# ska-telescope/ska-sdp-screen-fitting

Hardware: AMD Instinct MI355X
Metric: screen-slots/sec (ant×time×freq) + FITS-cube wall-clock, KL 256² screen (higher is better)
Workload: dtype f64

## Files before the change

### include/screenfit.h

```cpp
#ifndef SCREENFIT_H
#define SCREENFIT_H

#include <stddef.h>
#include <stdint.h>

#ifdef __cplusplus
extern "C" {
#endif

#define SF_OK 0
#define SF_EINVAL (-22)
#define SF_ENOMEM (-12)
#define SF_EIO (-5)
#define SF_ENODEV (-19)

#define SF_MAX_DIR 60
#define SF_MAX_FIT_DIR 128
#define SF_MAX_EVAL_DIR 128

#define SF_SCREEN_PHASE 0
#define SF_SCREEN_TEC 1
#define SF_SCREEN_AMPLITUDE 2

#define SF_EVAL_NAN_SCRUB 1u
// ... 32 lines not shown
#define SF_OPT_EVAL_XCD_MAP 7
#define SF_OPT_EVAL_GROUPS 8
#define SF_OPT_EVAL_BANDS 9
#define SF_OPT_FIT_LEAN 10
#define SF_OPT_TESS_SLOTS 11
#define SF_OPT_TESS_WAVES 12
#define SF_OPT_TESS_TILE 13
#define SF_OPT_TESS_BOX 14
#define SF_OPT_EVAL_INT 15
#define SF_OPT_EVAL_WG_WAVES 16
#define SF_OPT_FIT_EIG_WAVES 17
#define SF_OPT_FIT_SUBSET_DELETION 18
#define SF_OPT_FIT_WIDE_CACHE 19
#define SF_OPT_FIT_WIDE_POOL_MB 20
#define SF_OPT_FIT_WIDE_POOL_MAX 21
#define SF_EVAL_KERNEL_AUTO 0
#define SF_EVAL_KERNEL_TILE 1
#define SF_EVAL_KERNEL_LDS4 2
#define SF_EVAL_KERNEL_LDS8 3
#define SF_EVAL_KERNEL_LDS16 4
#define SF_EVAL_KERNEL_LDS8H 5
#define SF_EVAL_KERNEL_LDS16H 6
#define SF_EVAL_KERNEL_TILE3 7
#define SF_EVAL_KERNEL_SHB 8
#define SF_EVAL_KERNEL_WIDE 9
int sf_get_eval_kernel(sf_ctx* ctx, int gain, unsigned flags, int* kernel);
#define SF_EVAL_CONTRACTION_F64 0
#define SF_EVAL_CONTRACTION_I8_DIGITS 1
int sf_get_eval_contraction(sf_ctx* ctx, int gain, unsigned flags, int* contraction);
int sf_set_option(sf_ctx* ctx, int option, int value);
// ... 6 lines not shown
                 double beta);
int sf_set_basis_wide(sf_ctx* ctx, const double* pp_host, int D, double r0,
                      double beta);
int sf_get_basis(sf_ctx* ctx, double* c_host, double* pinv_c_host,
                 double* u_host, double* eig_host);

int sf_set_piercepoints(sf_ctx* ctx, const double* pp_host, int D, double r0,
                        double beta);

int sf_kl_fit(sf_ctx* ctx, const double* phase, const float* weight, int T,
              int F, int A, const int* station_order_host,
              const sf_fit_params* params, double* coef, double* resid,
              float* w_out, int32_t* order_out);

int sf_get_fit_stats(sf_ctx* ctx, int* n_masks, int* n_general);

int sf_get_fit_pool(sf_ctx* ctx, uint64_t* masks_host, double* entries_host,
                    int max_masks, int* n_masks);
int sf_get_fit_pool_wide(sf_ctx* ctx, uint64_t* masks_host, double* entries_host,
                         int max_masks, int* n_masks);

int sf_set_grid(sf_ctx* ctx, const double* x_host, int nx,
                const double* y_host, int ny);

int sf_kl_eval(sf_ctx* ctx, const double* coef, int64_t S, float* out,
               int64_t ring_slots, unsigned flags);

int sf_kl_eval_gain(sf_ctx* ctx, const double* coef_phase,
                    const double* coef_xx, const double* coef_yy, int64_t S,
                    float* out, int64_t ring_slots, unsigned flags);
// ... 33 lines not shown
```

### ska-sdp-screen-fitting_amd/csrc/capi.hip

```cpp
#include <hip/hip_runtime.h>

#include <algorithm>
#include <cmath>
#include <cstring>
#include <string>
#include <vector>

#include "sf_internal.h"

namespace sf {
static thread_local std::string g_last_error;
void set_error(const std::string& msg) { g_last_error = msg; }
}

using sf::set_error;

namespace {

int check_device(int device) {
  int n = 0;
  hipError_t e = hipGetDeviceCount(&n);
  if (e != hipSuccess || n == 0) {
    set_error("no HIP device available");
    return SF_ENODEV;
// ... 103 lines not shown
  hipFree(ctx->d_cfrag);
  hipFree(ctx->d_pxy);
  hipFree(ctx->d_pfrag);
  hipFree(ctx->d_cdig);
  hipFree(ctx->d_kdig);
  hipFree(ctx->d_kflag);
  if (ctx->kdig_read) (void)hipEventDestroy(ctx->kdig_read);
  hipFree(ctx->d_skip);
  hipFree(ctx->d_st_order);
  hipFree(ctx->d_keys);
  hipFree(ctx->d_ids);
  hipFree(ctx->d_pool_mask);
  hipFree(ctx->d_pool);
  hipFree(ctx->d_pool_status);
  hipFree(ctx->d_pos);
  hipFree(ctx->d_sigma);
  hipFree(ctx->d_class);
  hipFree(ctx->d_counters);
  hipFree(ctx->d_scratch);
  hipFree(ctx->d_wscratch);
  hipFree(ctx->d_oscratch);
  hipFree(ctx->d_gw);
  hipFree(ctx->d_smooth);
  hipFree(ctx->d_tess_tab);
  hipFree(ctx->d_tec_ch);
  hipFree(ctx->d_trash);
  delete ctx;
  return SF_OK;
}

// ... 46 lines not shown
  SF_REQUIRE(ctx, SF_EINVAL, "sf_set_option: NULL context");
  switch (option) {
    case SF_OPT_FIT_GENERAL:
      ctx->force_general = value != 0;
      return SF_OK;
    case SF_OPT_EVAL_KERNEL:
      SF_REQUIRE(value >= SF_EVAL_KERNEL_AUTO && value <= SF_EVAL_KERNEL_WIDE,
                 SF_EINVAL, "sf_set_option: unknown evaluation kernel");
      ctx->eval_kernel = value;
      return SF_OK;
    case SF_OPT_FIT_PACK:
      ctx->fit_pack = value != 0;
      return SF_OK;
    case SF_OPT_FIT_LEAN:
      ctx->fit_lean = value != 0;
      return SF_OK;
    case SF_OPT_EVAL_KS_PAD:
      SF_REQUIRE(value >= 0 && value <= 3, SF_EINVAL,
                 "sf_set_option: k-step padding must be 0..3");
      ctx->eval_ks_pad = value;
      return SF_OK;
    case SF_OPT_EVAL_SLEEP:
      SF_REQUIRE(value >= 0 && value <= 1000, SF_EINVAL,
                 "sf_set_option: eval sleep must be 0..1000");
      ctx->eval_sleep = value;
      return SF_OK;
    case SF_OPT_EVAL_XCD_MAP:
      SF_REQUIRE(value >= -1 && value <= 1, SF_EINVAL,
                 "sf_set_option: XCD map must be -1, 0 or 1");
      ctx->eval_xcd_map = value;
// ... 273 lines not shown
}

int sf_get_fit_stats(sf_ctx* ctx, int* n_masks, int* n_general) {
  SF_REQUIRE(ctx, SF_EINVAL, "sf_get_fit_stats: NULL context");
  int c[sf::kFitCounters] = {};
  SF_HIP(hipSetDevice(ctx->device));
  SF_HIP(hipStreamSynchronize(ctx->stream));
  if (ctx->d_counters)
    SF_HIP(hipMemcpy(c, ctx->d_counters, sizeof(c), hipMemcpyDeviceToHost));
  static_assert(sf::kCntIds == sf::kCntWideDecomp, "n_masks reads one slot");
  if (n_masks) *n_masks = c[sf::kCntIds];
  if (n_general) *n_general = c[sf::kCntSlow];
  return SF_OK;
}

int sf_get_fit_pool(sf_ctx* ctx, uint64_t* masks_host, double* entries_host,
                    int max_masks, int* n_masks) {
  SF_REQUIRE(ctx && n_masks && max_masks >= 0, SF_EINVAL, "sf_get_fit_pool: bad argument");
  SF_REQUIRE(max_masks == 0 || (masks_host && entries_host), SF_EINVAL,
             "sf_get_fit_pool: NULL output");
  SF_REQUIRE(!ctx->wide, SF_EINVAL,
             "sf_get_fit_pool: 64-bit mask keys; above SF_MAX_DIR directions "
             "(sf_set_basis_wide) call sf_get_fit_pool_wide");
  SF_HIP(hipSetDevice(ctx->device));
  SF_HIP(hipStreamSynchronize(ctx->stream));
  int c0 = 0;
  if (ctx->d_counters)
    SF_HIP(hipMemcpy(&c0, ctx->d_counters + sf::kCntIds, sizeof(int),
                     hipMemcpyDeviceToHost));
  const int n = ctx->pool_D == ctx->D && (size_t)c0 <= ctx->pool_cap ? c0 : 0;
// ... 392 lines not shown
```

### ska-sdp-screen-fitting_amd/csrc/kl_fit_fast.hip

```cpp
#include <hip/hip_runtime.h>

#include <cmath>
#include <cstdlib>

#include "kl_fit_pool.h"
#include "kl_fit_steps.h"
#include "sf_internal.h"

namespace sf {

constexpr size_t kLdsBytes = 160 * 1024;
constexpr double kTinyW = kPinvAtol * 1.001;

template <int GW>
__global__ __launch_bounds__(256) void kl_classify_kernel(
    const float* __restrict__ weight, int64_t S, int F, int A, int D,
    const int* __restrict__ st_order, const uint8_t* __restrict__ skip,
    int ref_skip, unsigned long long* __restrict__ keys, int cap,
    int* __restrict__ pos, uint8_t* __restrict__ cls,
    int* __restrict__ counters,
    double* __restrict__ coef, double* __restrict__ resid,
    float* __restrict__ w_out, int32_t* __restrict__ order_out) {
  constexpr int kPerWave = 64 / GW;
  const int l = lane();
// ... 227 lines not shown

#ifndef SF_FIT_MINW
#define SF_FIT_MINW 4
#endif
template <bool SLOW, int SPW, bool LEAN>
__global__ __launch_bounds__(256, SLOW ? 1 : SF_FIT_MINW) void kl_fit_pass_kernel(
    int it, int niter, int64_t S, int F, int A, int D,
    const double* __restrict__ phase, const double* __restrict__ refph,
    int ref_sub, const double* __restrict__ g_u, const double* __restrict__ g_c,
    const double* __restrict__ g_eig, const int* __restrict__ st_order,
    const uint8_t* __restrict__ cls, int* __restrict__ pos,
    const int* __restrict__ ids, unsigned long long* __restrict__ keys, int cap,
    const double* __restrict__ pool, int pool_cap, int* __restrict__ counters,
    int screen_type, double nsigma, int adjust_order, double* __restrict__ coef,
    double* __restrict__ resid, float* __restrict__ w_out,
    int32_t* __restrict__ order_out) {
#pragma clang fp contract(off)
  extern __shared__ double smem[];
  const int ld = odd_ld(D);
  using G = Group<SPW>;
  using M = FitMath<!SLOW>;
  const G tm;
  constexpr bool CG = SPW == 1;
  const int nwaves = blockDim.x / 64;
  const int nslots = nwaves * SPW;
  const int wv = (threadIdx.x / 64) * SPW + G::index();
  const int d = G::lane();
  double* sU = smem;
  double* sC = CG ? nullptr : sU + D * ld;
  double* sl = sU + (CG ? 1 : 2) * D * ld;
  for (int e = threadIdx.x; e < D * D; e += blockDim.x) {
// ... 13 lines not shown
    L.Vs = L.G = L.M = L.lams = nullptr;
    L.vec = wb;
    L.cs = nullptr;
    L.pr = nullptr;
  } else {
    L.Vs = wb;
    L.G = wb + D * ld;
    L.M = L.G + D * ld;
    L.lams = (SLOW ? L.M + D * ld : L.G + D * ld);
    L.vec = L.lams + 64;
    L.cs = reinterpret_cast<double2*>(L.vec + 6 * 64);
    L.pr = reinterpret_cast<int2*>(L.cs + 64);
  }
  const uint8_t want = SLOW ? 2 : 0;

  for (int64_t s = (int64_t)blockIdx.x * nslots + wv; s < S;
       s += (int64_t)gridDim.x * nslots) {
    if (SLOW && cls[s] != want) continue;
    const uint8_t cl = SLOW ? want : cls[s];
    const int a = (int)(s % A);
    const int p0 = pos[s];
    const int64_t base = s * D;
    double phi_d = 0.0, w_d = 0.0, white_d = 0.0, resid_d = 0.0;
    if (d < D) {
      phi_d = phase_ref(phase, refph, ref_sub, s, a, A, D, d);
      w_d = (double)w_out[base + d];
      white_d = it == 0 ? 0.0 : coef[base + d];
      resid_d = it == 0 ? 0.0 : resid[base + d];
    }
    double order = (double)order_out[s];
    const double station_order = (double)st_order[a];
    if (cl != want) continue;
// ... 150 lines not shown
    if (fabs(sd) > nsigma * sig && w != 0.0f) {
      w = 0.0f;
      w_out[s * D + d] = w;
      changed = true;
    }
    if (w > 0.0f) m |= 1ull << d;
  }
  if (changed) {
    pos[s] = (m == 0ull) ? -2 : (m == full_mask(D) ? -1 : table_insert(keys, cap, m));
  }
}

static int launch_pass(sf_ctx* ctx, bool slow, int it, const sf_fit_params* p,
                       const RefSpec& r, int64_t S, int F, int A,
                       const double* phase, double* coef, double* resid,
                       float* w_out, int32_t* order_out, bool lean) {
  const int D = ctx->D;
  const int spw = !slow && D <= 32 && ctx->fit_pack ? 2 : 1;
  lean = !slow && lean && ctx->fit_lean;
  decltype(&kl_fit_pass_kernel<false, 1, false>) const kernels[3][2] = {
      {kl_fit_pass_kernel<false, 1, false>, kl_fit_pass_kernel<false, 2, false>},
      {kl_fit_pass_kernel<false, 1, true>, kl_fit_pass_kernel<false, 2, true>},
      {kl_fit_pass_kernel<true, 1, false>, kl_fit_pass_kernel<true, 2, false>}};
  const auto kernel = kernels[slow ? 2 : lean][spw - 1];
  const size_t shared = fast_shared_bytes(D, spw == 1);
  const size_t slot = fast_wave_bytes(D, slow, lean);
  int nw = 1, best = 0;
  for (int k = 1; k <= 4; ++k) {
    const size_t per_wg = shared + (size_t)k * spw * slot;
    if (per_wg > kLdsBytes) break;
    const int waves = k * (int)(kLdsBytes / per_wg);
    if (waves > best) {
      best = waves;
      nw = k;
    }
  }
  const size_t shm = shared + (size_t)nw * spw * slot;
  SF_TRY_RC(allow_lds(kernel, shm));
  int64_t blocks = (S + nw * spw - 1) / (nw * spw);
  if (blocks > 16384) blocks = 16384;
  hipLaunchKernelGGL(kernel, dim3((unsigned)blocks), dim3(64 * nw), shm,
                     ctx->stream, it, p->niter, S, F, A, D, phase, r.refph, r.sub,
                     ctx->d_u, ctx->d_c, ctx->d_eig, ctx->d_st_order, ctx->d_class,
                     ctx->d_pos, ctx->d_ids, ctx->d_keys, (int)ctx->table_cap,
                     ctx->d_pool, (int)ctx->pool_cap, ctx->d_counters,
                     p->screen_type, p->nsigma, p->adjust_order, coef, resid, w_out,
                     order_out);
  SF_HIP(hipGetLastError());
  return SF_OK;
}

int launch_block_sigma(sf_ctx* ctx, int T, int F, int A, const double* phase,
                       const RefSpec& r, int screen_type, const double* resid,
                       const float* w_out) {
  hipLaunchKernelGGL(kl_block_sigma_kernel, dim3(F * A), dim3(256), 0,
                     ctx->stream, T, F, A, ctx->D, phase, r.refph, r.sub,
                     ctx->d_skip, r.skip, screen_type, resid, w_out,
                     ctx->d_sigma);
  SF_HIP(hipGetLastError());
  return SF_OK;
}

int fit_buffers(sf_ctx* ctx, int64_t S, int F, int A, double** resid,
// ... 39 lines not shown
  }
  SF_TRY_RC(fit_buffers(ctx, S, F, A, &resid, &w_out, &order_out));
  if (ctx->slot_cap < (size_t)S)
    SF_TRY_RC(replace_pair(ctx->slot_cap, (size_t)S, &ctx->d_pos, (size_t)S,
                           &ctx->d_class, (size_t)S));
  const size_t tcap = next_pow2((size_t)(2 * p->niter + 2) * (size_t)S + 64, 1);
  if (ctx->table_cap < tcap)
    SF_TRY_RC(replace_pair(ctx->table_cap, tcap, &ctx->d_keys, tcap, &ctx->d_ids, tcap));
  SF_TRY_RC(ensure_pool(ctx, 1024));
  const int cap = (int)ctx->table_cap;
  SF_HIP(hipMemsetAsync(ctx->d_keys, 0, ctx->table_cap * sizeof(unsigned long long),
                        ctx->stream));
  SF_HIP(hipMemsetAsync(ctx->d_ids, 0xff, ctx->table_cap * sizeof(int), ctx->stream));
  SF_HIP(hipMemsetAsync(ctx->d_counters, 0, kFitCounters * sizeof(int), ctx->stream));

  {
    const int gw = D <= 8 ? 8 : D <= 16 ? 16 : D <= 32 ? 32 : 64;
    const int64_t per_block = 4 * (64 / gw);
    const dim3 grid((unsigned)((S + per_block - 1) / per_block));
    const auto classify = gw == 8    ? kl_classify_kernel<8>
                          : gw == 16 ? kl_classify_kernel<16>
                          : gw == 32 ? kl_classify_kernel<32>
                                     : kl_classify_kernel<64>;
    hipLaunchKernelGGL(classify, grid, dim3(256), 0, ctx->stream, weight, S, F, A, D,
                       ctx->d_st_order, ctx->d_skip, r.skip, ctx->d_keys, cap,
                       ctx->d_pos, ctx->d_class, ctx->d_counters, coef, resid, w_out,
                       order_out);
    SF_HIP(hipGetLastError());
  }

  const bool block_flags = p->screen_type != SF_SCREEN_PHASE;
  for (int it = 0; it < p->niter; ++it) {
    int n_slow = 0, n_nonuniform = 0;
    SF_TRY_RC(number_and_decompose(ctx, &n_slow, &n_nonuniform));
    SF_TRY_RC(launch_pass(ctx, false, it, p, r, S, F, A, phase, coef, resid, w_out,
                          order_out, n_nonuniform == 0));
    if (n_slow > 0)
      SF_TRY_RC(launch_pass(ctx, true, it, p, r, S, F, A, phase, coef, resid, w_out,
                            order_out, false));
    if (block_flags && it + 1 < p->niter) {
      SF_TRY_RC(launch_block_sigma(ctx, T, F, A, phase, r, p->screen_type, resid,
                                 w_out));
      hipLaunchKernelGGL(kl_block_flag_kernel, dim3((unsigned)((S + 255) / 256)),
                         dim3(256), 0, ctx->stream, S, F, A, D, phase, r.refph,
                         r.sub, ctx->d_class, p->screen_type, p->nsigma,
                         ctx->d_sigma, resid, w_out, ctx->d_keys, cap,
                         ctx->d_pos);
// ... 20 lines not shown
```

### ska-sdp-screen-fitting_amd/csrc/kl_fit_pool.h

```cpp
#pragma once

#include <hip/hip_runtime.h>

#include <algorithm>

#include "kl_fit_masks.h"
#include "kl_fit_steps.h"
#include "sf_internal.h"

namespace sf {

constexpr unsigned long long kEmptyKey = 0ull;

__device__ int table_insert(unsigned long long* keys, int cap,
                            unsigned long long key) {
  int h = (int)(mix64(key) & (unsigned long long)(cap - 1));
  for (int probe = 0; probe < cap; ++probe) {
    unsigned long long prev = keys[h];
    if (prev == kEmptyKey) prev = atomicCAS(keys + h, kEmptyKey, key);
    if (prev == kEmptyKey || prev == key) return h;
    h = (h + 1) & (cap - 1);
  }
  return -3;
}
// ... 377 lines not shown
  SF_TRY_RC(grow(&ctx->d_pool_mask, mc, cap, true));
  ctx->pool_cap = cap;
  return SF_OK;
}

__global__ __launch_bounds__(256) void kl_fill_mask_kernel(
    const unsigned long long* __restrict__ keys, const int* __restrict__ ids,
    int cap, unsigned long long* __restrict__ pool_mask, int lo) {
  const int i = blockIdx.x * blockDim.x + threadIdx.x;
  if (i >= cap) return;
  if (keys[i] != kEmptyKey && ids[i] >= lo) pool_mask[ids[i]] = keys[i];
}

constexpr int kAncestorMinMasks = 8192;

static int number_and_decompose(sf_ctx* ctx, int* n_slow, int* n_nonuniform) {
  SF_HIP(hipMemcpyAsync(ctx->d_counters + kCntPassStart, ctx->d_counters + kCntIds,
                        sizeof(int), hipMemcpyDeviceToDevice, ctx->stream));
  SF_HIP(hipMemsetAsync(ctx->d_counters + kCntMaxLevel, 0, sizeof(int), ctx->stream));
  const int cap = (int)ctx->table_cap;
  const int old_cap = (int)ctx->pool_cap;
  hipLaunchKernelGGL(kl_assign_kernel, dim3(std::min((cap + 255) / 256, 8192)), dim3(256), 0,
                     ctx->stream, ctx->d_keys, cap, ctx->d_ids,
                     ctx->d_pool_mask, old_cap, ctx->d_counters, ctx->D);
  SF_HIP(hipGetLastError());
  int cnt[kCntMaxLevel + 1];
  SF_HIP(hipMemcpyAsync(cnt, ctx->d_counters, sizeof(cnt), hipMemcpyDeviceToHost,
                        ctx->stream));
  SF_HIP(hipStreamSynchronize(ctx->stream));
  *n_slow = cnt[kCntSlow];
  *n_nonuniform = cnt[kCntNonUniform];
  if (cnt[kCntIds] > old_cap) {
    SF_TRY_RC(ensure_pool(ctx, (size_t)cnt[kCntIds]));
    hipLaunchKernelGGL(kl_fill_mask_kernel, dim3((cap + 255) / 256), dim3(256),
                       0, ctx->stream, ctx->d_keys, ctx->d_ids, cap,
                       ctx->d_pool_mask, old_cap);
    SF_HIP(hipGetLastError());
  }
  const int n_new = cnt[kCntIds] - cnt[kCntPassStart];
  const uint8_t* done = nullptr;
  if (n_new > 0 && ctx->fit_subset_deletion && ctx->D <= 64) {
    SF_TRY_RC(grow(&ctx->d_pool_status, ctx->pool_status_cap, ctx->pool_cap, true));
    SF_HIP(hipMemsetAsync(ctx->d_pool_status + cnt[kCntPassStart], 1, (size_t)n_new, ctx->stream));
    const int D = ctx->D;
    const int ldd = odd_ld(D);
    const size_t shm = (size_t)2 * D * ldd * sizeof(double) + 6 * 64 * sizeof(double) +
// ... 36 lines not shown
```

### ska-sdp-screen-fitting_amd/csrc/sf_internal.h

```cpp
#pragma once

#include <hip/hip_runtime.h>

#include <cstdint>
#include <string>
#include <vector>

#include "screenfit.h"

namespace sf {

void set_error(const std::string& msg);

#define SF_HIP(call)                                                        \
  do {                                                                      \
    hipError_t e_ = (call);                                                 \
    if (e_ != hipSuccess) {                                                 \
      ::sf::set_error(std::string(#call) + ": " + hipGetErrorString(e_));   \
      return SF_EIO;                                                        \
    }                                                                       \
  } while (0)

#define SF_REQUIRE(cond, code, msg) \
  do {                              \
// ... 48 lines not shown
  if (shm > 64 * 1024)
    SF_HIP(hipFuncSetAttribute(reinterpret_cast<const void*>(kernel),
                               hipFuncAttributeMaxDynamicSharedMemorySize, (int)shm));
  return SF_OK;
}

enum FitCounter {
  kCntIds = 0,
  kCntWideDecomp = 0,
  kCntPassStart = 1,
  kCntSlow = 2,
  kCntError = 3,
  kCntNonUniform = 4,
  kCntMaxLevel = 5,
  kCntWideMasks = 6,
};
constexpr int kFitCounters = 8;
enum FitError {
  kErrLookupMiss = 1,
  kErrTableFull = 2,
  kErrLeanNonUniform = 4,
  kErrFullMaskInPool = 8,
};

constexpr int kTiles = 4;
constexpr int kWavePix = 16 * kTiles;
constexpr int kEvalWaves = 4;
constexpr int kBlockPix = kWavePix * kEvalWaves;

constexpr int kDigits = 6;

}
// ... 91 lines not shown
  size_t tess_tab_cap = 0;
  int force_general = 0;
  int eval_kernel = SF_EVAL_KERNEL_AUTO;
  int64_t eval_max_blocks = 0;
  int eval_ks_pad = 0;
  int eval_sleep = 0;
  int eval_xcd_map = -1;
  int eval_groups = 0;
  int eval_bands = 0;
  int tess_slots = 0;
  int tess_waves = 0;
  int tess_tile = 0;
  int tess_box = -1;
  int fit_pack = 1;
  int fit_lean = 1;
};

namespace sf {
constexpr int kEvalMaxKS = 15;
constexpr int kEvalWideMaxKS = SF_MAX_EVAL_DIR / 4;
inline bool eval_int_applies(const sf_ctx* ctx, bool gain, unsigned flags,
                             bool out_aligned16) {
  return !gain && ctx->dig_ok && ctx->d_cdig && ctx->eval_int != 0 &&
         (flags & SF_EVAL_FAST_SINCOS) && ctx->n_pix % 4 == 0 && out_aligned16 &&
         ctx->ksteps >= 12 && ctx->ksteps <= kEvalMaxKS;
}

struct RefSpec {
  int sub = -1;
  const double* refph = nullptr;
// ... 57 lines not shown
```

### ska-sdp-screen-fitting_amd/ska_sdp_screen_fitting_amd/_lib.py

```python

import contextlib
import ctypes
import os
import threading

import numpy as np

_HERE = os.path.dirname(os.path.abspath(__file__))
LIB_PATH = os.environ.get("SCREENFIT_LIB", os.path.join(_HERE, "libscreenfit.so"))

SF_SCREEN_PHASE = 0
SF_SCREEN_TEC = 1
SF_SCREEN_AMPLITUDE = 2
SF_EVAL_NAN_SCRUB = 1
SF_EVAL_FAST_SINCOS = 1 << 8
SF_EVAL_NT_STORES = 1 << 9
SF_EVAL_BIG_ENDIAN = 1 << 10
SF_MAX_DIR = 60
SF_MAX_FIT_DIR = 128
SF_MAX_EVAL_DIR = 128
SF_MAX_POINTS = 4096
SF_MAX_TEC_FREQ = 4096
SF_OPT_FIT_GENERAL = 1
SF_OPT_EVAL_KERNEL = 2
# ... 4 lines not shown
SF_OPT_EVAL_XCD_MAP = 7
SF_OPT_EVAL_GROUPS = 8
SF_OPT_EVAL_BANDS = 9
SF_OPT_FIT_LEAN = 10
SF_OPT_TESS_SLOTS = 11
SF_OPT_TESS_WAVES = 12
SF_OPT_TESS_TILE = 13
SF_OPT_TESS_BOX = 14
SF_OPT_EVAL_INT = 15
SF_OPT_EVAL_WG_WAVES = 16
SF_OPT_FIT_EIG_WAVES = 17
SF_OPT_FIT_SUBSET_DELETION = 18
SF_OPT_FIT_WIDE_CACHE = 19
SF_OPT_FIT_WIDE_POOL_MB = 20
SF_OPT_FIT_WIDE_POOL_MAX = 21
SF_EVAL_KERNEL_AUTO = 0
SF_EVAL_KERNEL_TILE = 1
SF_EVAL_KERNEL_LDS4 = 2
SF_EVAL_KERNEL_LDS8 = 3
SF_EVAL_KERNEL_LDS16 = 4
SF_EVAL_KERNEL_LDS8H = 5
SF_EVAL_KERNEL_LDS16H = 6
SF_EVAL_KERNEL_TILE3 = 7
SF_EVAL_KERNEL_SHB = 8
SF_EVAL_KERNEL_WIDE = 9
EVAL_KERNEL_NAMES = {SF_EVAL_KERNEL_TILE: "kl_eval_kernel",
                     SF_EVAL_KERNEL_LDS4: "kl_eval_lds_kernel<4 waves>",
                     SF_EVAL_KERNEL_LDS8: "kl_eval_lds_kernel<8 waves>",
                     SF_EVAL_KERNEL_LDS16: "kl_eval_lds_kernel<16 waves>",
                     SF_EVAL_KERNEL_LDS8H: "kl_eval_lds_kernel<8 waves, 2 tiles>",
                     SF_EVAL_KERNEL_LDS16H: "kl_eval_lds_kernel<16 waves, 2 tiles>",
                     SF_EVAL_KERNEL_TILE3: "kl_eval_kernel<3 waves/SIMD>",
                     SF_EVAL_KERNEL_SHB: "kl_eval_kernel<Cpix in LDS>",
                     SF_EVAL_KERNEL_WIDE: "kl_eval_wide_kernel"}

EXPORTED = (
    "sf_version", "sf_last_error", "sf_create", "sf_destroy", "sf_set_stream",
    "sf_synchronize", "sf_set_option", "sf_get_eval_kernel", "sf_get_eval_contraction", "sf_alloc", "sf_free", "sf_copy_h2d", "sf_copy_d2h",
    "sf_set_basis", "sf_set_basis_wide", "sf_set_piercepoints", "sf_get_basis", "sf_kl_fit", "sf_get_fit_stats", "sf_get_fit_pool",
    "sf_get_fit_pool_wide",
    "sf_stream_create", "sf_stream_destroy", "sf_device_cus",
    "sf_set_grid", "sf_kl_eval", "sf_kl_eval_gain", "sf_kl_eval_sums",
    "sf_tess_fill", "sf_smooth",
    "sf_set_points", "sf_kl_eval_points", "sf_kl_eval_point_values",
    "sf_kl_eval_values",
    "sf_set_tec_freqs", "sf_kl_eval_tec",
)


_identity = {}


def library_identity(path=None):
    import hashlib
# ... 46 lines not shown
            "sf_synchronize": ([vp], c_int),
            "sf_set_option": ([vp, c_int, c_int], c_int),
            "sf_get_eval_kernel": ([vp, c_int, ctypes.c_uint, ip], c_int),
            "sf_get_eval_contraction": ([vp, c_int, ctypes.c_uint, ip], c_int),
            "sf_alloc": ([vp, ctypes.c_size_t, ctypes.POINTER(vp)], c_int),
            "sf_free": ([vp, vp], c_int),
            "sf_copy_h2d": ([vp, vp, vp, ctypes.c_size_t], c_int),
            "sf_copy_d2h": ([vp, vp, vp, ctypes.c_size_t], c_int),
            "sf_set_basis": ([vp, vp, c_int, c_dbl, c_dbl], c_int),
            "sf_set_basis_wide": ([vp, vp, c_int, c_dbl, c_dbl], c_int),
            "sf_set_piercepoints": ([vp, vp, c_int, c_dbl, c_dbl], c_int),
            "sf_get_basis": ([vp, vp, vp, vp, vp], c_int),
            "sf_kl_fit": ([vp, vp, vp, c_int, c_int, c_int, ip,
                           ctypes.POINTER(FitParams), vp, vp, vp, vp], c_int),
            "sf_get_fit_stats": ([vp, ip, ip], c_int),
            "sf_get_fit_pool": ([vp, vp, vp, c_int, ip], c_int),
            "sf_get_fit_pool_wide": ([vp, vp, vp, c_int, ip], c_int),
            "sf_set_grid": ([vp, vp, c_int, vp, c_int], c_int),
            "sf_kl_eval": ([vp, vp, i64, vp, i64, ctypes.c_uint], c_int),
            "sf_stream_create": ([vp, ctypes.POINTER(c_int), c_int,
                                  ctypes.POINTER(vp)], c_int),
            "sf_stream_destroy": ([vp, vp], c_int),
            "sf_device_cus": ([vp, ctypes.POINTER(c_int)], c_int),
            "sf_kl_eval_gain": ([vp, vp, vp, vp, i64, vp, i64, ctypes.c_uint],
                                c_int),
            "sf_kl_eval_sums": ([vp, vp, vp, vp, i64, vp, i64, ctypes.c_uint, vp],
                                c_int),
            "sf_tess_fill": ([vp, vp, c_int, c_int, vp, vp, vp, c_int, i64, vp,
                              i64, c_dbl, ctypes.c_uint], c_int),
            "sf_smooth": ([vp, vp, c_int, c_int, i64, c_dbl, ctypes.c_uint], c_int),
# ... 154 lines not shown
            self.h, self._dev(phase, np.float64, n, "phase"),
            self._dev(weight, np.float32, n, "weight"), int(T), int(F), int(A),
            so.ctypes.data_as(ctypes.POINTER(ctypes.c_int)),
            ctypes.byref(prm), self._dev(coef, np.float64, n, "coef"),
            self._dev(resid, np.float64, n, "resid"),
            self._dev(w_out, np.float32, n, "w_out"),
            self._dev(order_out, np.int32, n // max(self.D, 1), "order_out")),
            "sf_kl_fit")

    def fit_stats(self):
        nm, ng = ctypes.c_int(), ctypes.c_int()
        _check(self.lib.sf_get_fit_stats(self.h, ctypes.byref(nm), ctypes.byref(ng)),
               "sf_get_fit_stats")
        return {"n_masks": nm.value, "n_general": ng.value}

    def fit_pool(self):
        n = ctypes.c_int(0)
        _check(self.lib.sf_get_fit_pool(self.h, None, None, 0, ctypes.byref(n)),
               "sf_get_fit_pool")
        D = self.D
        masks = np.zeros(n.value, np.uint64)
        ent = np.zeros((n.value, D * D + D))
        if n.value:
            _check(self.lib.sf_get_fit_pool(self.h, masks.ctypes.data, ent.ctypes.data,
                                            n.value, ctypes.byref(n)), "sf_get_fit_pool")
        order = np.argsort(masks, kind="stable")
        masks, ent = masks[order], ent[order]
        for k, m in enumerate(masks):
            n = bin(int(m)).count("1")
            u = ent[k, :D * D].reshape(D, D)
# ... 198 lines not shown
```

Baseline: 6.175 million.

## Add lane-per-slot fit path with compacted work lists for phase screens

Adds a new KL fit path for phase screens with D between 3 and 24. A front kernel fits one slot per lane, using a padded basis in global memory and LDS tiles. Each iteration a check kernel decides per slot whether it is finished, and only the slots that still need the general pass are appended to a compacted list via ballot and atomics. The existing pass kernel then iterates over that list instead of all slots. The aim is to skip redundant per-slot work and replace wave-per-slot processing with a lane-per-slot layout, at the cost of extra kernels, register pressure from DP-sized arrays, and a new numerical path that must match the old results.

```diff
diff --git a/include/screenfit.h b/include/screenfit.h
--- a/include/screenfit.h
+++ b/include/screenfit.h
@@ -70,6 +70,7 @@
 #define SF_OPT_FIT_WIDE_CACHE 19
 #define SF_OPT_FIT_WIDE_POOL_MB 20
 #define SF_OPT_FIT_WIDE_POOL_MAX 21
+#define SF_OPT_FIT_LANE 22
 #define SF_EVAL_KERNEL_AUTO 0
 #define SF_EVAL_KERNEL_TILE 1
 #define SF_EVAL_KERNEL_LDS4 2
@@ -106,6 +107,8 @@
               float* w_out, int32_t* order_out);
 
 int sf_get_fit_stats(sf_ctx* ctx, int* n_masks, int* n_general);
+int sf_get_fit_lane_stats(sf_ctx* ctx, int* n_passes, int* finished, int* listed,
+                          int max_passes);
 
 int sf_get_fit_pool(sf_ctx* ctx, uint64_t* masks_host, double* entries_host,
                     int max_masks, int* n_masks);
diff --git a/ska-sdp-screen-fitting_amd/csrc/capi.hip b/ska-sdp-screen-fitting_amd/csrc/capi.hip
--- a/ska-sdp-screen-fitting_amd/csrc/capi.hip
+++ b/ska-sdp-screen-fitting_amd/csrc/capi.hip
@@ -141,6 +141,8 @@
   hipFree(ctx->d_pool);
   hipFree(ctx->d_pool_status);
   hipFree(ctx->d_pos);
+  hipFree(ctx->d_lane_list);
+  hipFree(ctx->d_lane_basis);
   hipFree(ctx->d_sigma);
   hipFree(ctx->d_class);
   hipFree(ctx->d_counters);
@@ -217,6 +219,9 @@
       return SF_OK;
     case SF_OPT_FIT_LEAN:
       ctx->fit_lean = value != 0;
+      return SF_OK;
+    case SF_OPT_FIT_LANE:
+      ctx->fit_lane = value != 0;
       return SF_OK;
     case SF_OPT_EVAL_KS_PAD:
       SF_REQUIRE(value >= 0 && value <= 3, SF_EINVAL,
@@ -520,6 +525,21 @@
   return SF_OK;
 }
 
+int sf_get_fit_lane_stats(sf_ctx* ctx, int* n_passes, int* finished, int* listed,
+                          int max_passes) {
+  SF_REQUIRE(ctx && n_passes && max_passes >= 0, SF_EINVAL,
+             "sf_get_fit_lane_stats: bad argument");
+  SF_REQUIRE(max_passes == 0 || (finished && listed), SF_EINVAL,
+             "sf_get_fit_lane_stats: NULL output");
+  const int n = (int)ctx->lane_finished.size();
+  *n_passes = n;
+  for (int i = 0; i < n && i < max_passes; ++i) {
+    finished[i] = ctx->lane_finished[i];
+    listed[i] = ctx->lane_listed[i];
+  }
+  return SF_OK;
+}
+
 int sf_get_fit_pool(sf_ctx* ctx, uint64_t* masks_host, double* entries_host,
                     int max_masks, int* n_masks) {
   SF_REQUIRE(ctx && n_masks && max_masks >= 0, SF_EINVAL, "sf_get_fit_pool: bad argument");
diff --git a/ska-sdp-screen-fitting_amd/csrc/kl_fit_fast.hip b/ska-sdp-screen-fitting_amd/csrc/kl_fit_fast.hip
--- a/ska-sdp-screen-fitting_amd/csrc/kl_fit_fast.hip
+++ b/ska-sdp-screen-fitting_amd/csrc/kl_fit_fast.hip
@@ -3,6 +3,7 @@
 #include <cmath>
 #include <cstdlib>
 
+#include "kl_fit_lane.h"
 #include "kl_fit_pool.h"
 #include "kl_fit_steps.h"
 #include "sf_internal.h"
@@ -265,7 +266,8 @@
     const double* __restrict__ pool, int pool_cap, int* __restrict__ counters,
     int screen_type, double nsigma, int adjust_order, double* __restrict__ coef,
     double* __restrict__ resid, float* __restrict__ w_out,
-    int32_t* __restrict__ order_out) {
+    int32_t* __restrict__ order_out, const int* __restrict__ list,
+    const int* __restrict__ list_count) {
 #pragma clang fp contract(off)
   extern __shared__ double smem[];
   const int ld = odd_ld(D);
@@ -309,8 +311,10 @@
   }
   const uint8_t want = SLOW ? 2 : 0;
 
-  for (int64_t s = (int64_t)blockIdx.x * nslots + wv; s < S;
-       s += (int64_t)gridDim.x * nslots) {
+  const int64_t n_items = list ? (int64_t)*list_count : S;
+  for (int64_t i = (int64_t)blockIdx.x * nslots + wv; i < n_items;
+       i += (int64_t)gridDim.x * nslots) {
+    const int64_t s = list ? (int64_t)list[i] : i;
     if (SLOW && cls[s] != want) continue;
     const uint8_t cl = SLOW ? want : cls[s];
     const int a = (int)(s % A);
@@ -491,7 +495,8 @@
 static int launch_pass(sf_ctx* ctx, bool slow, int it, const sf_fit_params* p,
                        const RefSpec& r, int64_t S, int F, int A,
                        const double* phase, double* coef, double* resid,
-                       float* w_out, int32_t* order_out, bool lean) {
+                       float* w_out, int32_t* order_out, bool lean,
+                       const int* list = nullptr, int n_list = 0) {
   const int D = ctx->D;
   const int spw = !slow && D <= 32 && ctx->fit_pack ? 2 : 1;
   lean = !slow && lean && ctx->fit_lean;
@@ -514,7 +519,8 @@
   }
   const size_t shm = shared + (size_t)nw * spw * slot;
   SF_TRY_RC(allow_lds(kernel, shm));
-  int64_t blocks = (S + nw * spw - 1) / (nw * spw);
+  const int64_t n_items = list ? n_list : S;
+  int64_t blocks = (n_items + nw * spw - 1) / (nw * spw);
   if (blocks > 16384) blocks = 16384;
   hipLaunchKernelGGL(kernel, dim3((unsigned)blocks), dim3(64 * nw), shm,
                      ctx->stream, it, p->niter, S, F, A, D, phase, r.refph, r.sub,
@@ -522,8 +528,61 @@
                      ctx->d_pos, ctx->d_ids, ctx->d_keys, (int)ctx->table_cap,
                      ctx->d_pool, (int)ctx->pool_cap, ctx->d_counters,
                      p->screen_type, p->nsigma, p->adjust_order, coef, resid, w_out,
-                     order_out);
+                     order_out, list, ctx->d_counters + kCntLaneList);
   SF_HIP(hipGetLastError());
+  return SF_OK;
+}
+
+static int launch_fit_lane(sf_ctx* ctx, const double* phase, const float* weight,
+                           int64_t S, int F, int A, const sf_fit_params* p,
+                           const RefSpec& r, double* coef, double* resid,
+                           float* w_out, int32_t* order_out) {
+  const int D = ctx->D;
+  const int cap = (int)ctx->table_cap;
+  SF_TRY_RC(grow(&ctx->d_lane_list, ctx->lane_list_cap, (size_t)S));
+  SF_TRY_RC(grow(&ctx->d_lane_basis, ctx->lane_basis_cap, kLaneBasisDoubles));
+  const dim3 grid((unsigned)((S + 63) / 64));
+  const int dp = lane_pad(D);
+  const auto front = dp == 8    ? kl_fit_lane_front_kernel<8>
+                     : dp == 16 ? kl_fit_lane_front_kernel<16>
+                     : dp == 20 ? kl_fit_lane_front_kernel<20>
+                                : kl_fit_lane_front_kernel<24>;
+  const auto check = dp == 8    ? kl_fit_lane_check_kernel<8>
+                     : dp == 16 ? kl_fit_lane_check_kernel<16>
+                     : dp == 20 ? kl_fit_lane_check_kernel<20>
+                                : kl_fit_lane_check_kernel<24>;
+  hipLaunchKernelGGL(kl_lane_basis_kernel, dim3(1), dim3(256), 0, ctx->stream, ctx->d_u,
+                     ctx->d_eig, D, dp, ctx->d_lane_basis);
+  SF_HIP(hipGetLastError());
+  hipLaunchKernelGGL(front, grid, dim3(64), lane_front_bytes(D), ctx->stream, p->niter,
+                     S, F, A, D, phase, weight, r.refph, r.sub, ctx->d_lane_basis,
+                     ctx->d_st_order, ctx->d_skip, r.skip, ctx->d_keys, cap, ctx->d_pos,
+                     ctx->d_class, ctx->d_counters, ctx->d_lane_list, kTinyW, p->nsigma,
+                     coef, resid, w_out, order_out);
+  SF_HIP(hipGetLastError());
+  bool lean = false;
+  for (int it = 0; it < p->niter; ++it) {
+    if (it > 0) {
+      SF_HIP(hipMemsetAsync(ctx->d_counters + kCntLaneList, 0, 2 * sizeof(int),
+                            ctx->stream));
+      hipLaunchKernelGGL(check, grid, dim3(64), lane_check_bytes(D), ctx->stream, it,
+                         p->niter, S, A, D, ctx->d_st_order, ctx->d_class, ctx->d_pos,
+                         ctx->d_keys, cap, ctx->d_counters, ctx->d_lane_list, p->nsigma,
+                         p->adjust_order, (int)lean, resid, w_out, order_out);
+      SF_HIP(hipGetLastError());
+    }
+    int n_slow = 0, n_nonuniform = 0, lane[2] = {0, 0};
+    SF_TRY_RC(number_and_decompose(ctx, &n_slow, &n_nonuniform, lane));
+    lean = n_nonuniform == 0 && ctx->fit_lean;
+    ctx->lane_listed.push_back(lane[0]);
+    ctx->lane_finished.push_back(lane[1]);
+    if (lane[0] > 0)
+      SF_TRY_RC(launch_pass(ctx, false, it, p, r, S, F, A, phase, coef, resid, w_out,
+                            order_out, n_nonuniform == 0, ctx->d_lane_list, lane[0]));
+    if (n_slow > 0)
+      SF_TRY_RC(launch_pass(ctx, true, it, p, r, S, F, A, phase, coef, resid, w_out,
+                            order_out, false));
+  }
   return SF_OK;
 }
 
@@ -593,7 +652,14 @@
   SF_HIP(hipMemsetAsync(ctx->d_ids, 0xff, ctx->table_cap * sizeof(int), ctx->stream));
   SF_HIP(hipMemsetAsync(ctx->d_counters, 0, kFitCounters * sizeof(int), ctx->stream));
 
-  {
+  ctx->lane_listed.clear();
+  ctx->lane_finished.clear();
+  const bool lane_path = ctx->fit_lane && p->screen_type == SF_SCREEN_PHASE &&
+                         D >= kLaneMinD && D <= kLaneMaxD;
+  if (lane_path) {
+    SF_TRY_RC(launch_fit_lane(ctx, phase, weight, S, F, A, p, r, coef, resid, w_out,
+                              order_out));
+  } else {
     const int gw = D <= 8 ? 8 : D <= 16 ? 16 : D <= 32 ? 32 : 64;
     const int64_t per_block = 4 * (64 / gw);
     const dim3 grid((unsigned)((S + per_block - 1) / per_block));
@@ -609,7 +675,7 @@
   }
 
   const bool block_flags = p->screen_type != SF_SCREEN_PHASE;
-  for (int it = 0; it < p->niter; ++it) {
+  for (int it = 0; it < p->niter && !lane_path; ++it) {
     int n_slow = 0, n_nonuniform = 0;
     SF_TRY_RC(number_and_decompose(ctx, &n_slow, &n_nonuniform));
     SF_TRY_RC(launch_pass(ctx, false, it, p, r, S, F, A, phase, coef, resid, w_out,
diff --git a/ska-sdp-screen-fitting_amd/csrc/kl_fit_lane.h b/ska-sdp-screen-fitting_amd/csrc/kl_fit_lane.h
--- /dev/null
+++ b/ska-sdp-screen-fitting_amd/csrc/kl_fit_lane.h
@@ -0,0 +1,447 @@
+#pragma once
+
+#include <hip/hip_runtime.h>
+
+#include <cmath>
+
+#include "kl_fit_pool.h"
+#include "kl_fit_steps.h"
+#include "sf_internal.h"
+
+namespace sf {
+
+constexpr int kLaneMinD = 3;
+constexpr int kLaneMaxD = 24;
+__host__ __device__ inline int lane_pad(int D) {
+  return D <= 8 ? 8 : D <= 16 ? 16 : D <= 20 ? 20 : 24;
+}
+constexpr size_t kLaneBasisDoubles = 2 * kLaneMaxD * kLaneMaxD + kLaneMaxD;
+
+__host__ __device__ inline size_t lane_tile(int D) { return (size_t)64 * odd_ld(D); }
+__host__ __device__ inline size_t lane_front_bytes(int D) {
+  return 2 * lane_tile(D) * sizeof(double);
+}
+__host__ __device__ inline size_t lane_check_bytes(int D) {
+  return 2 * lane_tile(D) * sizeof(double) + lane_tile(D) * sizeof(float);
+}
+
+__global__ __launch_bounds__(256) void kl_lane_basis_kernel(
+    const double* __restrict__ g_u, const double* __restrict__ g_eig, int D, int DP,
+    double* __restrict__ ub) {
+  for (int e = threadIdx.x; e < D * DP; e += blockDim.x) {
+    const int p = e / DP, l = e % DP;
+    ub[e] = l < D ? g_u[p * D + l] : 0.0;
+    ub[D * DP + e] = l < D ? g_u[l * D + p] : 0.0;
+  }
+  for (int l = threadIdx.x; l < DP; l += blockDim.x)
+    ub[2 * D * DP + l] = l < D ? g_eig[l] : 0.0;
+}
+
+template <int DP, class Leaf>
+__device__ __forceinline__ double lane_tree_sum(int D, Leaf leaf) {
+#pragma clang fp contract(off)
+  double x[32];
+#pragma unroll
+  for (int i = 0; i < 32; ++i) {
+    x[i] = 0.0;
+    if (i < DP) {
+      const double v = leaf(i < D ? i : 0);
+      x[i] = i < D ? v : 0.0;
+    }
+  }
+#pragma unroll
+  for (int o = 16; o > 0; o >>= 1) {
+#pragma unroll
+    for (int i = 0; i < o; ++i) x[i] = x[i] + x[i + o];
+  }
+  return x[0];
+}
+
+__device__ __forceinline__ void lane_append(bool on, int64_t s, int* counter,
+                                            int* __restrict__ list) {
+  const unsigned long long m = __ballot(on);
+  if (m == 0ull) return;
+  int base = 0;
+  if (lane() == 0) base = atomicAdd(counter, __popcll(m));
+  base = __shfl(base, 0);
+  if (on) list[base + Group<1>::rank(m)] = (int)s;
+}
+
+__device__ __forceinline__ void lane_count(bool on, int* counter) {
+  const unsigned long long m = __ballot(on);
+  if (m != 0ull && lane() == 0) atomicAdd(counter, __popcll(m));
+}
+
+template <class Op>
+__device__ __forceinline__ void lane_tile_walk(int D, int ld, int nel, Op op) {
+  const int l = lane();
+  int r = l / D, c = l % D;
+  const int dr = 64 / D, dc = 64 % D;
+  for (int e = l; e < nel; e += 64) {
+    op(e, r * ld + c);
+    r += dr;
+    c += dc;
+    if (c >= D) {
+      c -= D;
+      ++r;
+    }
+  }
+}
+
+template <int DP, class M, class NonZero>
+__device__ __forceinline__ unsigned lane_outliers(int D, double nsigma, double* R,
+                                                  double* X, NonZero nonzero) {
+#pragma clang fp contract(off)
+  double cnt = 0.0;
+  for (int d = 0; d < D; ++d) {
+    double r = M::mod(R[d], 2.0 * M_PI);
+    if (r < -M_PI) r += 2.0 * M_PI;
+    if (r > M_PI) r -= 2.0 * M_PI;
+    const bool inc = nonzero(d) && !isnan(r);
+    double sn = 0.0, cn = 0.0;
+    if (inc) M::sin_cos(r, &sn, &cn);
+    R[d] = r;
+    X[d] = sn;
+    cnt += inc ? 1.0 : 0.0;
+  }
+  const double t1 = lane_tree_sum<DP>(D, [&](int i) { return X[i]; });
+  for (int d = 0; d < D; ++d) {
+    const double r = R[d];
+    double sn = 0.0, cn = 0.0;
+    if (nonzero(d) && !isnan(r)) M::sin_cos(r, &sn, &cn);
+    X[d] = cn;
+  }
+  const double t2 = lane_tree_sum<DP>(D, [&](int i) { return X[i]; });
+  const double ms = t1 / cnt;
+  const double mc = t2 / cnt;
+  const double stdv = sqrt(-2.0 * M::ln(hypot(ms, mc)));
+  const double thr = nsigma * stdv;
+  unsigned out = 0u;
+  for (int d = 0; d < D; ++d)
+    if (fabs(R[d]) > thr) out |= 1u << d;
+  return out;
+}
+
+template <int DP, class M>
+__device__ __forceinline__ void lane_fit_once(const double* __restrict__ ub, int D,
+                                              int K, int Kmax, double wu, double* X,
+                                              double* Y, double (&wh)[DP],
+                                              double (&cw)[DP]) {
+#pragma clang fp contract(off)
+  const double* __restrict__ ut = ub + D * DP;
+  const double* __restrict__ lam = ut + D * DP;
+  for (int p = 0; p < D; ++p) {
+    double sn, cn;
+    M::sin_cos(X[p], &sn, &cn);
+    X[p] = wu * cn;
+    Y[p] = wu * sn;
+  }
+  {
+    double a1[DP], a2[DP];
+#pragma unroll
+    for (int l = 0; l < DP; ++l) a1[l] = a2[l] = 0.0;
+    for (int p = 0; p < D; ++p) {
+      const double xp = X[p], yp = Y[p];
+      const double* ur = ub + p * DP;
+#pragma unroll
+      for (int l = 0; l < DP; ++l) {
+        const double u = ur[l];
+        a1[l] += u * xp;
+        a2[l] += u * yp;
+      }
+    }
+#pragma unroll
+    for (int l = 0; l < DP; ++l) {
+      const bool keep = fabs(lam[l]) > kPinvAtol;
+      const double q1 = a1[l] / wu;
+      const double q2 = a2[l] / wu;
+      if (l < Kmax) {
+        X[l] = keep ? q1 : 0.0;
+        Y[l] = keep ? q2 : 0.0;
+      }
+    }
+  }
+  {
+    double cr[DP], ci[DP];
+#pragma unroll
+    for (int l = 0; l < DP; ++l) cr[l] = ci[l] = 0.0;
+    for (int k = 0; k < Kmax; ++k) {
+      if (k < K) {
+        const double xk = X[k], yk = Y[k];
+        const double* uc = ut + k * DP;
+#pragma unroll
+        for (int l = 0; l < DP; ++l) {
+          const double u = uc[l];
+          cr[l] += u * xk;
+          ci[l] += u * yk;
+        }
+      }
+    }
+#pragma unroll
+    for (int l = 0; l < DP; ++l)
+      if (l < D) {
+        X[l] = cr[l];
+        Y[l] = ci[l];
+      }
+  }
+  for (int p = 0; p < D; ++p) X[p] = M::arctan2(Y[p], X[p]);
+  {
+    double sh[DP];
+#pragma unroll
+    for (int l = 0; l < DP; ++l) sh[l] = 0.0;
+    for (int p = 0; p < D; ++p) {
+      const double xp = X[p];
+      const double* ur = ub + p * DP;
+#pragma unroll
+      for (int l = 0; l < DP; ++l) sh[l] += ur[l] * xp;
+    }
+#pragma unroll
+    for (int l = 0; l < DP; ++l) {
+      const double lm = lam[l];
+      const bool keep = fabs(lm) > kPinvAtol;
+      const double q = sh[l] / lm;
+      if (l < D) {
+        X[l] = keep ? q : 0.0;
+        Y[l] = keep ? sh[l] : 0.0;
+      }
+    }
+  }
+#pragma unroll
+  for (int l = 0; l < DP; ++l) wh[l] = cw[l] = 0.0;
+  for (int r = 0; r < D; ++r) {
+    const double xr = X[r], yr = Y[r];
+    const double* uc = ut + r * DP;
+#pragma unroll
+    for (int l = 0; l < DP; ++l) {
+      const double u = uc[l];
+      wh[l] += u * xr;
+      cw[l] += u * yr;
+    }
+  }
+}
+
+template <int DP>
+__global__ __launch_bounds__(64) void kl_fit_lane_front_kernel(
+    int niter, int64_t S, int F, int A, int D, const double* __restrict__ phase,
+    const float* __restrict__ weight, const double* __restrict__ refph,
+    int ref_sub, const double* __restrict__ ub, const int* __restrict__ st_order,
+    const uint8_t* __restrict__ skip, int ref_skip,
+    unsigned long long* __restrict__ keys, int cap, int* __restrict__ pos,
+    uint8_t* __restrict__ cls, int* __restrict__ counters, int* __restrict__ list,
+    double tiny_w, double nsigma, double* __restrict__ coef,
+    double* __restrict__ resid, float* __restrict__ w_out,
+    int32_t* __restrict__ order_out) {
+#pragma clang fp contract(off)
+  extern __shared__ double smem[];
+  using M = FitMath<false>;
+  const int ld = odd_ld(D);
+  const int l = lane();
+  double* tX = smem;
+  double* tY = tX + lane_tile(D);
+  float* tW = reinterpret_cast<float*>(tY);
+  const int64_t s0 = (int64_t)blockIdx.x * 64;
+  const int ns = (int)(S - s0 < 64 ? S - s0 : 64);
+  const int nel = ns * D;
+  const int64_t e0 = s0 * D;
+  lane_tile_walk(D, ld, nel, [&](int e, int at) {
+    tX[at] = phase[e0 + e];
+    const float w = weight[e0 + e];
+    w_out[e0 + e] = w;
+    tW[at] = w;
+  });
+  lds_sync();
+
+  const int64_t s = s0 + l;
+  const bool valid = l < ns;
+  const unsigned full = (unsigned)full_mask(D);
+  int a = 0;
+  bool skipped = false, tiny = false, nonuniform = false;
+  unsigned mask = 0u;
+  float wf = 0.0f;
+  if (valid) {
+    const SlotGeom sg(s, F, A);
+    a = sg.a;
+    skipped = sg.skipped(skip, ref_skip);
+    const float* wr = tW + l * ld;
+    for (int d = 0; d < D; ++d) {
+      const float x = wr[d];
+      if (x > 0.0f) {
+        if (mask == 0u) wf = x;
+        mask |= 1u << d;
+        if ((double)x <= tiny_w) tiny = true;
+        if (x != wf) nonuniform = true;
+      }
+    }
+  }
+  lds_sync();
+  const bool fitted = valid && !skipped;
+  const bool elig = fitted && !tiny && mask == full && !nonuniform;
+  int ord = 0, K = 0;
+  if (fitted) ord = st_order[a];
+  if (elig) K = ord < D - 1 ? ord : D - 1;
+  int km = K;
+#pragma unroll
+  for (int o = 32; o > 0; o >>= 1) km = max(km, __shfl_xor(km, o, 64));
+  const int Kmax = __builtin_amdgcn_readfirstlane(km);
+  lane_count(fitted && tiny, counters + kCntSlow);
+  lane_count(fitted && !tiny && nonuniform, counters + kCntNonUniform);
+
+  double* X = tX + l * ld;
+  double* Y = tY + l * ld;
+  double wh[DP], res[DP];
+#pragma unroll
+  for (int i = 0; i < DP; ++i) wh[i] = res[i] = 0.0;
+  if (elig) {
+    for (int d = 0; d < D; ++d) {
+      double v = X[d];
+      if (refph) v -= refph[(s / A) * D + d];
+      else if (ref_sub >= 0) v -= phase[(s + (ref_sub - a)) * D + d];
+      X[d] = v;
+    }
+    double phi[DP], cw[DP];
+#pragma unroll
+    for (int i = 0; i < DP; ++i) phi[i] = X[i < D ? i : 0];
+    lane_fit_once<DP, M>(ub, D, K, Kmax, (double)wf, X, Y, wh, cw);
+#pragma unroll
+    for (int i = 0; i < DP; ++i) res[i] = phi[i] - cw[i];
+  }
+#pragma unroll
+  for (int i = 0; i < DP; ++i)
+    if (i < D) {
+      X[i] = wh[i];
+      Y[i] = res[i];
+    }
+  lds_sync();
+  lane_tile_walk(D, ld, nel, [&](int e, int at) {
+    coef[e0 + e] = tX[at];
+    resid[e0 + e] = tY[at];
+  });
+  lds_sync();
+
+  int p_new = -1;
+  if (elig && niter > 1) {
+    const unsigned out = lane_outliers<DP, M>(D, nsigma, Y, X, [](int) { return true; });
+    if (out != 0u) {
+      asm volatile("s_waitcnt vmcnt(0)" ::: "memory");
+      for (int d = 0; d < D; ++d)
+        if ((out >> d) & 1u) w_out[s * D + d] = 0.0f;
+      const unsigned nm = full & ~out;
+      p_new = nm == 0u ? -2 : table_insert(keys, cap, (unsigned long long)nm);
+    }
+  }
+  if (valid) {
+    if (skipped) {
+      cls[s] = 1;
+      order_out[s] = 0;
+      pos[s] = -2;
+    } else {
+      cls[s] = tiny ? 2 : 0;
+      order_out[s] = elig ? K : ord;
+      if (elig) pos[s] = p_new;
+      else if (mask == full) pos[s] = -1;
+      else if (mask == 0u) pos[s] = -2;
+      else pos[s] = table_insert(keys, cap, (unsigned long long)mask);
+    }
+  }
+  lane_count(elig, counters + kCntLaneDone);
+  lane_append(fitted && !tiny && !elig, s, counters + kCntLaneList, list);
+}
+
+template <int DP>
+__global__ __launch_bounds__(64) void kl_fit_lane_check_kernel(
+    int it, int niter, int64_t S, int A, int D, const int* __restrict__ st_order,
+    const uint8_t* __restrict__ cls, int* __restrict__ pos,
+    unsigned long long* __restrict__ keys, int cap, int* __restrict__ counters,
+    int* __restrict__ list, double nsigma, int adjust_order, int lean,
+    const double* __restrict__ resid, float* __restrict__ w_out,
+    int32_t* __restrict__ order_out) {
+#pragma clang fp contract(off)
+  extern __shared__ double smem[];
+  using M = FitMath<false>;
+  const int ld = odd_ld(D);
+  const int l = lane();
+  double* tX = smem;
+  double* tR = tX + lane_tile(D);
+  float* tW = reinterpret_cast<float*>(tR + lane_tile(D));
+  const int64_t s0 = (int64_t)blockIdx.x * 64;
+  const int ns = (int)(S - s0 < 64 ? S - s0 : 64);
+  const int nel = ns * D;
+  const int64_t e0 = s0 * D;
+  lane_tile_walk(D, ld, nel, [&](int e, int at) {
+    tR[at] = resid[e0 + e];
+    tW[at] = w_out[e0 + e];
+  });
+  lds_sync();
+
+  const int64_t s = s0 + l;
+  const bool mine = l < ns && cls[s] == 0;
+  double* X = tX + l * ld;
+  double* R = tR + l * ld;
+  const float* W = tW + l * ld;
+  bool listed = false, done = false;
+  if (mine) {
+    const int p0 = pos[s];
+    const int ord0 = order_out[s];
+    const double station_order = (double)st_order[(int)(s % A)];
+    double order = (double)ord0;
+    int n_unfl = 0;
+    double wmax = -INFINITY, wmin = INFINITY;
+    for (int d = 0; d < D; ++d) {
+      const double w = (double)W[d];
+      if (w > 0.0) {
+        ++n_unfl;
+        wmax = fmax(wmax, w);
+        wmin = fmin(wmin, w);
+      }
+    }
+    listed = p0 == -3 || (lean && n_unfl > 0 && wmax != wmin);
+    if (!listed && n_unfl > 0) {
+      if (order > n_unfl - 1) order = n_unfl - 1;
+      if (adjust_order) {
+        const double r0 = lane_tree_sum<DP>(D, [&](int i) {
+          const double w = (double)W[i];
+          return w > 0.0 ? w : 0.0;
+        });
+        double r12[2];
+#pragma unroll
+        for (int h = 0; h < 2; ++h) {
+          for (int d = 0; d < D; ++d) {
+            const double w = (double)W[d];
+            const bool unfl = w > 0.0;
+            double sn = 0.0, cn = 0.0;
+            if (unfl) M::sin_cos(R[d], &sn, &cn);
+            const double ww = unfl ? w : 0.0;
+            X[d] = h == 0 ? sn * sn * ww : cn * cn * ww;
+          }
+          r12[h] = lane_tree_sum<DP>(D, [&](int i) { return X[i]; });
+        }
+        const double m1 = r12[0] / r0;
+        const double m2 = r12[1] / r0;
+        const double redchi2 = (1.0 - hypot(m1, m2)) * r0 / (n_unfl - order);
+        OrderWalk walk;
+        double moved = order;
+        listed = !walk.template step<M>(0, redchi2, n_unfl, station_order, moved);
+      }
+    }
+    if (!listed) {
+      done = true;
+      if (it + 1 < niter && n_unfl > 0) {
+        const unsigned out = lane_outliers<DP, M>(
+            D, nsigma, R, X, [&](int d) { return (double)W[d] != 0.0; });
+        if (out != 0u) {
+          unsigned nm = 0u;
+          for (int d = 0; d < D; ++d) {
+            if ((out >> d) & 1u) w_out[s * D + d] = 0.0f;
+            else if ((double)W[d] > 0.0) nm |= 1u << d;
+          }
+          pos[s] = nm == 0u ? -2 : table_insert(keys, cap, (unsigned long long)nm);
+        }
+      }
+      if ((int32_t)order != ord0) order_out[s] = (int32_t)order;
+    }
+  }
+  lane_count(done, counters + kCntLaneDone);
+  lane_append(listed, s, counters + kCntLaneList, list);
+}
+
+}
diff --git a/ska-sdp-screen-fitting_amd/csrc/kl_fit_pool.h b/ska-sdp-screen-fitting_amd/csrc/kl_fit_pool.h
--- a/ska-sdp-screen-fitting_amd/csrc/kl_fit_pool.h
+++ b/ska-sdp-screen-fitting_amd/csrc/kl_fit_pool.h
@@ -415,7 +415,8 @@
 
 constexpr int kAncestorMinMasks = 8192;
 
-static int number_and_decompose(sf_ctx* ctx, int* n_slow, int* n_nonuniform) {
+static int number_and_decompose(sf_ctx* ctx, int* n_slow, int* n_nonuniform,
+                                int* lane = nullptr) {
   SF_HIP(hipMemcpyAsync(ctx->d_counters + kCntPassStart, ctx->d_counters + kCntIds,
                         sizeof(int), hipMemcpyDeviceToDevice, ctx->stream));
   SF_HIP(hipMemsetAsync(ctx->d_counters + kCntMaxLevel, 0, sizeof(int), ctx->stream));
@@ -425,12 +426,16 @@
                      ctx->stream, ctx->d_keys, cap, ctx->d_ids,
                      ctx->d_pool_mask, old_cap, ctx->d_counters, ctx->D);
   SF_HIP(hipGetLastError());
-  int cnt[kCntMaxLevel + 1];
+  int cnt[kFitCounters];
   SF_HIP(hipMemcpyAsync(cnt, ctx->d_counters, sizeof(cnt), hipMemcpyDeviceToHost,
                         ctx->stream));
   SF_HIP(hipStreamSynchronize(ctx->stream));
   *n_slow = cnt[kCntSlow];
   *n_nonuniform = cnt[kCntNonUniform];
+  if (lane) {
+    lane[0] = cnt[kCntLaneList];
+    lane[1] = cnt[kCntLaneDone];
+  }
   if (cnt[kCntIds] > old_cap) {
     SF_TRY_RC(ensure_pool(ctx, (size_t)cnt[kCntIds]));
     hipLaunchKernelGGL(kl_fill_mask_kernel, dim3((cap + 255) / 256), dim3(256),
diff --git a/ska-sdp-screen-fitting_amd/csrc/sf_internal.h b/ska-sdp-screen-fitting_amd/csrc/sf_internal.h
--- a/ska-sdp-screen-fitting_amd/csrc/sf_internal.h
+++ b/ska-sdp-screen-fitting_amd/csrc/sf_internal.h
@@ -86,8 +86,10 @@
   kCntNonUniform = 4,
   kCntMaxLevel = 5,
   kCntWideMasks = 6,
-};
-constexpr int kFitCounters = 8;
+  kCntLaneList = 7,
+  kCntLaneDone = 8,
+};
+constexpr int kFitCounters = 10;
 enum FitError {
   kErrLookupMiss = 1,
   kErrTableFull = 2,
@@ -209,6 +211,12 @@
   int tess_box = -1;
   int fit_pack = 1;
   int fit_lean = 1;
+  int fit_lane = 1;
+  int* d_lane_list = nullptr;
+  size_t lane_list_cap = 0;
+  double* d_lane_basis = nullptr;
+  size_t lane_basis_cap = 0;
+  std::vector<int> lane_finished, lane_listed;
 };
 
 namespace sf {
diff --git a/ska-sdp-screen-fitting_amd/ska_sdp_screen_fitting_amd/_lib.py b/ska-sdp-screen-fitting_amd/ska_sdp_screen_fitting_amd/_lib.py
--- a/ska-sdp-screen-fitting_amd/ska_sdp_screen_fitting_amd/_lib.py
+++ b/ska-sdp-screen-fitting_amd/ska_sdp_screen_fitting_amd/_lib.py
@@ -42,6 +42,7 @@
 SF_OPT_FIT_WIDE_CACHE = 19
 SF_OPT_FIT_WIDE_POOL_MB = 20
 SF_OPT_FIT_WIDE_POOL_MAX = 21
+SF_OPT_FIT_LANE = 22
 SF_EVAL_KERNEL_AUTO = 0
 SF_EVAL_KERNEL_TILE = 1
 SF_EVAL_KERNEL_LDS4 = 2
@@ -65,7 +66,7 @@
 EXPORTED = (
     "sf_version", "sf_last_error", "sf_create", "sf_destroy", "sf_set_stream",
     "sf_synchronize", "sf_set_option", "sf_get_eval_kernel", "sf_get_eval_contraction", "sf_alloc", "sf_free", "sf_copy_h2d", "sf_copy_d2h",
-    "sf_set_basis", "sf_set_basis_wide", "sf_set_piercepoints", "sf_get_basis", "sf_kl_fit", "sf_get_fit_stats", "sf_get_fit_pool",
+    "sf_set_basis", "sf_set_basis_wide", "sf_set_piercepoints", "sf_get_basis", "sf_kl_fit", "sf_get_fit_stats", "sf_get_fit_lane_stats", "sf_get_fit_pool",
     "sf_get_fit_pool_wide",
     "sf_stream_create", "sf_stream_destroy", "sf_device_cus",
     "sf_set_grid", "sf_kl_eval", "sf_kl_eval_gain", "sf_kl_eval_sums",
@@ -142,6 +143,7 @@
             "sf_kl_fit": ([vp, vp, vp, c_int, c_int, c_int, ip,
                            ctypes.POINTER(FitParams), vp, vp, vp, vp], c_int),
             "sf_get_fit_stats": ([vp, ip, ip], c_int),
+            "sf_get_fit_lane_stats": ([vp, ip, ip, ip, c_int], c_int),
             "sf_get_fit_pool": ([vp, vp, vp, c_int, ip], c_int),
             "sf_get_fit_pool_wide": ([vp, vp, vp, c_int, ip], c_int),
             "sf_set_grid": ([vp, vp, c_int, vp, c_int], c_int),
@@ -326,6 +328,16 @@
                "sf_get_fit_stats")
         return {"n_masks": nm.value, "n_general": ng.value}
 
+    def fit_lane_stats(self):
+        n = ctypes.c_int(0)
+        fin = (ctypes.c_int * 64)()
+        lst = (ctypes.c_int * 64)()
+        _check(self.lib.sf_get_fit_lane_stats(self.h, ctypes.byref(n), fin, lst, 64),
+               "sf_get_fit_lane_stats")
+        k = n.value
+        return {"front": fin[0] if k else 0, "checked": list(fin[1:k]),
+                "listed": list(lst[:k])}
+
     def fit_pool(self):
         n = ctypes.c_int(0)
         _check(self.lib.sf_get_fit_pool(self.h, None, None, 0, ctypes.byref(n)),
```

New measurement: 6.228 million, median of 6. No clear change (+0.9%).
